# victorramirez952/tomography_3d_reconstructor

Hardware: AMD Instinct MI355X
Metric: Mvoxels/s (SDF+MC) on 1024^3 ellipsoid stack; achieved HBM GB/s vs peak (higher is better)
Workload: dtype f64

## Files before the change

### include/tomo_hip.h

```cpp
#ifndef TOMO_HIP_H
#define TOMO_HIP_H

#include <stddef.h>
#include <stdint.h>

#ifdef __cplusplus
extern "C" {
#endif

#define TOMO_OK 0
#define TOMO_E_ARG (-1)
#define TOMO_E_LAUNCH (-2)
#define TOMO_E_SIZE (-3)
#define TOMO_E_WORKSPACE (-4)

int tomo_abi_version(void);
const char *tomo_error_string(int code);
int tomo_host_mc_cell(const float *h_v, double iso, int8_t *h_tris, int *h_uses_centre);
double tomo_host_mc_edge_offset(double va, double vb);
void tomo_host_mc_centre_offset(const double *h_v8, double *h_out3);

int tomo_host_checksum(const void *h_data, int64_t nbytes, int nthreads, uint64_t *h_out);
int tomo_host_checksum_impl(const void *h_data, int64_t nbytes, int nthreads, int impl, uint64_t *h_out);
int64_t tomo_host_checksum_chunk_bytes(void);
// ... 57 lines not shown
int tomo_field_signs(const float *field, int Nz, int Ny, int Nx, int64_t pitch, int xorg, double iso, int z_begin,
                     int z_end, unsigned long long *signs, uint8_t *gcls, void *stream);

int tomo_mc_classify(const unsigned long long *signs, const uint8_t *gcls, int Nz, int Ny, int Nx, int xorg,
                     unsigned long long *seg_act, uint32_t *seg_cnt, void *stream);
int tomo_mc_scan_segments(const uint32_t *seg_cnt, int64_t nseg, uint32_t *seg_aoff, unsigned long long *totals,
                          void *workspace, int64_t workspace_bytes, void *stream);
int64_t tomo_mc_scan_workspace_bytes(int64_t n);
int tomo_mc_scan(const uint32_t *counts, int64_t n, uint32_t *off_a, uint32_t *off_b, uint32_t *nz_ids,
                 unsigned long long *totals, void *workspace, int64_t workspace_bytes, void *stream);
int tomo_mc_list(int Nz, int Ny, int Nx, int xorg, const uint32_t *seg_aoff, const unsigned long long *seg_act,
                 unsigned long long *vox_key, void *stream);
int tomo_mc_eval(const float *field, int Nz, int Ny, int Nx, int64_t pitch, int xorg, double iso,
                 const unsigned long long *vox_key, int64_t na, uint32_t *vox_counts, uint8_t *vox_flags, void *stream);
int tomo_mc_list_capped(int Nz, int Ny, int Nx, int xorg, const uint32_t *seg_aoff, const unsigned long long *seg_act,
                        unsigned long long *vox_key, int64_t cap, void *stream);
int tomo_mc_eval_capped(const float *field, int Nz, int Ny, int Nx, int64_t pitch, int xorg, double iso,
                        const unsigned long long *vox_key, int64_t cap, const unsigned long long *na_dev,
                        uint32_t *vox_counts, uint8_t *vox_flags, void *stream);
int tomo_mc_emit(const float *field, int Nz, int Ny, int Nx, int64_t pitch, int xorg, double iso,
                 const unsigned long long *vox_key, int64_t na, const unsigned long long *seg_act,
                 const uint32_t *seg_aoff, const uint32_t *vox_voff, const uint32_t *vox_foff, const uint8_t *vox_flags,
                 int z_offset, unsigned long long *vkey, float *vpos, int32_t *faces, unsigned long long *totals,
                 void *stream);

int tomo_mc_first_touch(const float *field, int Nz, int Ny, int Nx, int64_t pitch, int xorg, double iso,
                        const unsigned long long *vox_key, int64_t na, const unsigned long long *seg_act,
                        const uint32_t *seg_aoff, const uint32_t *vox_voff, const uint8_t *vox_flags, int mode,
                        uint32_t *created, const uint32_t *base, int32_t *ft_rank, unsigned long long *totals, void *stream);

int tomo_mc3_list(int Nz, int Ny, int Nx, int xorg, const uint32_t *seg_cnt, const unsigned long long *seg_act,
                  uint32_t *seg_blk, uint32_t *seg_aoff, unsigned long long *vox_key, int64_t cap, unsigned long long *tot,
                  void *stream);
int tomo_mc3_eval(const float *field, int Nz, int Ny, int Nx, int64_t pitch, int xorg, double iso,
                  const unsigned long long *vox_key, int64_t cap, const unsigned long long *tot, int z_offset,
                  uint32_t *vox_loc, int32_t *vox_til, uint8_t *vox_flags, uint16_t *vox_used, float *vox_f3, float *vox_c3,
                  uint32_t *blk3, void *stream);
int64_t tomo_mc3_slice_table_words(int Nz, int Ny);
int64_t tomo_mc3_sort_segments(int Nz, int Ny);
int tomo_mc3_scan(int Nz, int Ny, int Nx, int xorg, const uint32_t *seg_aoff, const uint32_t *vox_loc, int64_t cap,
                  uint32_t *blk3, uint32_t *slice_tab, unsigned long long *tot, int64_t cap_v, int64_t cap_f, void *stream);
int tomo_mc3_vertices(int Nz, int Ny, int Nx, int xorg, const unsigned long long *vox_key, int64_t cap,
                      const unsigned long long *tot, const uint32_t *vox_loc, const uint8_t *vox_flags, const float *vox_f3,
                      const float *vox_c3, const uint32_t *blk3, const uint32_t *slice_tab, int z_offset, int shift,
                      const double *cum, int64_t ncum, const double *adj, int64_t nadj, float mm_y, float mm_x, float *vrec,
                      uint32_t *keys, uint32_t *idx, void *stream);
int64_t tomo_mc3_sort_workspace_bytes(int64_t cap_v, int64_t nseg);
int tomo_mc3_sort_rank_top(const float *vrec, uint32_t *keys, uint32_t *idx, int64_t cap_v, int Nz, int Ny, const uint32_t *slice_tab,
                           unsigned long long *tot, float *uniq, int32_t *table, void *workspace, int64_t workspace_bytes,
                           float z_top, void *stream);
int tomo_mc3_sort_rank_fused(const float *vrec, const uint32_t *keys, int64_t cap_v, int Nz, int Ny, uint32_t *slice_tab,
                             unsigned long long *tot, float *uniq, int32_t *table, float z_top, void *stream);
int tomo_mc3_faces(int Nz, int Ny, int Nx, int xorg, const unsigned long long *vox_key, int64_t cap, unsigned long long *tot,
                   const unsigned long long *seg_act, const uint32_t *seg_aoff, const uint32_t *vox_loc, const int32_t *vox_til,
                   const uint16_t *vox_used, const uint32_t *blk3, const int32_t *table, int64_t *faces, int64_t cap_f,
                   void *stream);

int tomo_vertex_finalize(float *vpos, int64_t nv, int shift, const double *cum, int64_t ncum,
                         const double *adj, int64_t nadj, float mm_y, float mm_x, void *stream);
int64_t tomo_mesh_unique_workspace_bytes(int64_t nv);
int tomo_mesh_unique(const float *vpos, int64_t nv, float *uniq, int32_t *rank, unsigned long long *totals,
                     void *workspace, int64_t workspace_bytes, void *stream);
int tomo_mesh_lookup(const float *uniq, int64_t nu, const float *query, int64_t nq, int32_t *out,
                     unsigned long long *missing, void *stream);
int tomo_slab_top_rows(const float *uniq, const unsigned long long *tot, int64_t cap_v, int64_t cap, float *msg, void *stream);
int tomo_slab_lookup(const float *uniq, const unsigned long long *tot, int64_t cap_v, const float *msg, int64_t cap,
// ... 42 lines not shown
```

### tomography_3d_reconstructor_amd/_lib.py

```python
import ctypes
import os
import subprocess

_HERE = os.path.dirname(os.path.abspath(__file__))
SO_PATH = os.environ.get("TOMO_LIB") or os.path.join(_HERE, "libtomo_hip.so")
CSRC = os.path.join(_HERE, "csrc")

_c_i = ctypes.c_int
_c_i64 = ctypes.c_int64
_c_p = ctypes.c_void_p
_c_d = ctypes.c_double
_c_f = ctypes.c_float

SIGNATURES = {
    "tomo_abi_version": (_c_i, []),
    "tomo_error_string": (ctypes.c_char_p, [_c_i]),
    "tomo_host_mc_cell": (_c_i, [_c_p, _c_d, _c_p, _c_p]),
    "tomo_host_mc_edge_offset": (_c_d, [_c_d, _c_d]),
    "tomo_host_mc_centre_offset": (None, [_c_p, _c_p]),
    "tomo_host_checksum": (_c_i, [_c_p, _c_i64, _c_i, _c_p]),
    "tomo_host_checksum_impl": (_c_i, [_c_p, _c_i64, _c_i, _c_i, _c_p]),
    "tomo_host_checksum_chunk_bytes": (_c_i64, []),
    "tomo_host_checksum_part": (_c_i, [_c_p, _c_i64, _c_i64, _c_i, _c_i, _c_p]),
    "tomo_host_checksum_fold": (_c_i, [_c_p, _c_i64, _c_i64, _c_p]),
# ... 24 lines not shown
    "tomo_pack_close_ends": (_c_i, [_c_p, _c_p, _c_i, _c_i, _c_i, _c_p, _c_p]),
    "tomo_pack_bits_pair": (_c_i, [_c_p, _c_p, _c_i, _c_p, _c_p, _c_i, _c_i, _c_i, _c_p]),
    "tomo_slab_edges": (_c_i, [_c_p, _c_p, _c_i, _c_i, _c_i, _c_i, _c_p, _c_p, _c_i, _c_i, _c_p, _c_p, _c_p, _c_i, _c_p, _c_p, _c_p, _c_p,
                               _c_i, _c_p, _c_p]),
    "tomo_pack_close_range": (_c_i, [_c_p, _c_p, _c_i, _c_i, _c_i, _c_i, _c_i, _c_p, _c_p, _c_i, _c_i, _c_p]),
    "tomo_close_ends_workspace_words": (_c_i64, [_c_i, _c_i, _c_i]),
    "tomo_close_ends_scan": (_c_i, [_c_p, _c_i, _c_i, _c_i, _c_p, _c_p]),
    "tomo_close_ends_gp": (_c_i, [_c_p, _c_i, _c_i, _c_i, _c_p, _c_p, _c_p]),
    "tomo_morph_pass": (_c_i, [_c_p, _c_p, _c_i, _c_i, _c_i, _c_i, _c_p]),
    "tomo_morph_fused": (_c_i, [_c_p, _c_p, _c_i, _c_i, _c_i, ctypes.c_uint32, _c_i, _c_p]),
    "tomo_smooth": (_c_i, [_c_p, _c_p, _c_i, _c_i, _c_i, _c_i, _c_i, _c_p]),
    "tomo_extend_bits": (_c_i, [_c_p, _c_p, _c_i, _c_i, _c_i, _c_i, _c_p]),
    "tomo_field_fill": (_c_i, [_c_p, _c_p, _c_i, _c_i, _c_i, _c_i, _c_i, _c_p, _c_p, _c_p]),
    "tomo_field_fill_bits": (_c_i, [_c_p, _c_p, _c_i, _c_i, _c_i, _c_i, _c_p, _c_p, _c_p]),
    "tomo_field_span_bytes": (_c_i64, [_c_i, _c_i, _c_i, _c_i]),
    "tomo_field_fill_bits_sparse": (_c_i, [_c_p, _c_p, _c_i, _c_i, _c_i, _c_i, _c_p, _c_p, _c_p, _c_p]),
    "tomo_sign_rows": (_c_i64, [_c_i]),
    "tomo_field_signs_fused": (_c_i, [_c_i]),
    "tomo_sign_buffer_words": (_c_i64, [_c_i, _c_i, _c_i, _c_i]),
    "tomo_field_signs": (_c_i, [_c_p, _c_i, _c_i, _c_i, _c_i64, _c_i, _c_d, _c_i, _c_i, _c_p, _c_p, _c_p]),
    "tomo_mc_classify": (_c_i, [_c_p, _c_p, _c_i, _c_i, _c_i, _c_i, _c_p, _c_p, _c_p]),
    "tomo_mc_scan_segments": (_c_i, [_c_p, _c_i64, _c_p, _c_p, _c_p, _c_i64, _c_p]),
    "tomo_mc_scan_workspace_bytes": (_c_i64, [_c_i64]),
    "tomo_mc_scan": (_c_i, [_c_p, _c_i64, _c_p, _c_p, _c_p, _c_p, _c_p, _c_i64, _c_p]),
    "tomo_mc_list": (_c_i, [_c_i, _c_i, _c_i, _c_i, _c_p, _c_p, _c_p, _c_p]),
    "tomo_mc_eval": (_c_i, [_c_p, _c_i, _c_i, _c_i, _c_i64, _c_i, _c_d, _c_p, _c_i64, _c_p, _c_p, _c_p]),
    "tomo_mc_list_capped": (_c_i, [_c_i, _c_i, _c_i, _c_i, _c_p, _c_p, _c_p, _c_i64, _c_p]),
    "tomo_mc_eval_capped": (_c_i, [_c_p, _c_i, _c_i, _c_i, _c_i64, _c_i, _c_d, _c_p, _c_i64, _c_p, _c_p, _c_p, _c_p]),
    "tomo_mc_emit": (_c_i, [_c_p, _c_i, _c_i, _c_i, _c_i64, _c_i, _c_d, _c_p, _c_i64, _c_p, _c_p, _c_p, _c_p, _c_p, _c_i, _c_p,
                            _c_p, _c_p, _c_p, _c_p]),
    "tomo_mc_first_touch": (_c_i, [_c_p, _c_i, _c_i, _c_i, _c_i64, _c_i, _c_d, _c_p, _c_i64, _c_p, _c_p, _c_p, _c_p, _c_i, _c_p,
                                   _c_p, _c_p, _c_p, _c_p]),
    "tomo_mc3_list": (_c_i, [_c_i, _c_i, _c_i, _c_i, _c_p, _c_p, _c_p, _c_p, _c_p, _c_i64, _c_p, _c_p]),
    "tomo_mc3_eval": (_c_i, [_c_p, _c_i, _c_i, _c_i, _c_i64, _c_i, _c_d, _c_p, _c_i64, _c_p, _c_i, _c_p, _c_p, _c_p, _c_p, _c_p,
                             _c_p, _c_p, _c_p]),
    "tomo_mc3_slice_table_words": (_c_i64, [_c_i, _c_i]),
    "tomo_mc3_sort_segments": (_c_i64, [_c_i, _c_i]),
    "tomo_mc3_scan": (_c_i, [_c_i, _c_i, _c_i, _c_i, _c_p, _c_p, _c_i64, _c_p, _c_p, _c_p, _c_i64, _c_i64, _c_p]),
    "tomo_mc3_vertices": (_c_i, [_c_i, _c_i, _c_i, _c_i, _c_p, _c_i64, _c_p, _c_p, _c_p, _c_p, _c_p, _c_p, _c_p, _c_i, _c_i,
                                 _c_p, _c_i64, _c_p, _c_i64, _c_f, _c_f, _c_p, _c_p, _c_p, _c_p]),
    "tomo_mc3_sort_workspace_bytes": (_c_i64, [_c_i64, _c_i64]),
    "tomo_mc3_sort_rank_top": (_c_i, [_c_p, _c_p, _c_p, _c_i64, _c_i, _c_i, _c_p, _c_p, _c_p, _c_p, _c_p, _c_i64, _c_f, _c_p]),
    "tomo_mc3_sort_rank_fused": (_c_i, [_c_p, _c_p, _c_i64, _c_i, _c_i, _c_p, _c_p, _c_p, _c_p, _c_f, _c_p]),
    "tomo_mc3_faces": (_c_i, [_c_i, _c_i, _c_i, _c_i, _c_p, _c_i64, _c_p, _c_p, _c_p, _c_p, _c_p, _c_p, _c_p, _c_p, _c_p, _c_i64, _c_p]),
    "tomo_vertex_finalize": (_c_i, [_c_p, _c_i64, _c_i, _c_p, _c_i64, _c_p, _c_i64, _c_f, _c_f, _c_p]),
    "tomo_mesh_unique_workspace_bytes": (_c_i64, [_c_i64]),
    "tomo_mesh_unique": (_c_i, [_c_p, _c_i64, _c_p, _c_p, _c_p, _c_p, _c_i64, _c_p]),
    "tomo_mesh_lookup": (_c_i, [_c_p, _c_i64, _c_p, _c_i64, _c_p, _c_p, _c_p]),
    "tomo_slab_top_rows": (_c_i, [_c_p, _c_p, _c_i64, _c_i64, _c_p, _c_p]),
    "tomo_slab_lookup": (_c_i, [_c_p, _c_p, _c_i64, _c_p, _c_i64, _c_p, _c_p, _c_p]),
    "tomo_slab_summary": (_c_i, [_c_p, _c_i64, _c_p, _c_p, _c_i64, _c_i64, _c_p, _c_p]),
    "tomo_slab_lookup_summary": (_c_i, [_c_p, _c_p, _c_i64, _c_p, _c_i64, _c_p, _c_i64, _c_i64, _c_p, _c_p, _c_p]),
    "tomo_mc3_faces_slab": (_c_i, [_c_i, _c_i, _c_i, _c_i, _c_p, _c_i64, _c_p, _c_p, _c_p, _c_p, _c_p, _c_p, _c_p, _c_p, _c_p, _c_i64,
                                   _c_p, _c_i, _c_i, _c_p, _c_i64, _c_i64, _c_p]),
    "tomo_mesh_volume_area": (_c_i, [_c_p, _c_p, _c_i64, _c_p, _c_p]),
    "tomo_layer_colors": (_c_i, [_c_p, _c_i, _c_i64, _c_i64, _c_d, _c_d, _c_i, _c_d, _c_d, _c_i, _c_p, _c_p]),
    "tomo_mesh_edge_table_bytes": (_c_i64, [_c_i64]),
    "tomo_mesh_edges": (_c_i, [_c_p, _c_i64, _c_i64, _c_p, _c_i64, _c_p, _c_p]),
    "tomo_mesh_seam_edges": (_c_i, [_c_p, _c_i64, _c_i64, _c_i64, _c_p, _c_i64, _c_p, _c_p]),
    "tomo_mesh_seam_merge": (_c_i, [_c_p, _c_i64, _c_i64, _c_p, _c_i64, _c_p, _c_p]),
    "tomo_mesh_orient_workspace_bytes": (_c_i64, [_c_i64]),
    "tomo_mesh_orient": (_c_i, [_c_p, _c_i64, _c_i64, _c_p, _c_i64, _c_p, _c_p, _c_p]),
    "tomo_mesh_signed_volume": (_c_i, [_c_p, _c_p, _c_i64, _c_p, _c_p, _c_p]),
    "tomo_glb_pack_faces": (_c_i, [_c_p, _c_i64, _c_p, _c_p, _c_p, _c_i, _c_p]),
    "tomo_glb_pack_positions": (_c_i, [_c_p, _c_i, _c_i64, _c_p, _c_p, _c_p]),
    "tomo_mesh_vertex_normals_workspace_bytes": (_c_i64, [_c_i64, _c_i64]),
# ... 49 lines not shown
```

### tomography_3d_reconstructor_amd/csrc/mc.hip

```cpp
#include <cstring>
#include <cstdlib>
#include "tomo_common.h"
#include <rocprim/rocprim.hpp>

#define MC_LUT_QUAL __device__ const
#define MC_FN __device__ static inline
#include "mc_cell.h"

#define SEG 256
#define KEY_XBITS 20
static_assert(KEY_XBITS + 2 == TOMO_KEY_ROW_SHIFT, "key layout shared with mesh.hip");

struct McGrid {
    int Nz, Ny, Nx;
    int64_t pitch;
    int xorg;
    int segs_per_row;
    double iso;
};

typedef float float4u __attribute__((ext_vector_type(4), aligned(4)));
typedef float float2u __attribute__((ext_vector_type(2), aligned(4)));
typedef float float3u __attribute__((ext_vector_type(3), aligned(4)));
typedef int int3u __attribute__((ext_vector_type(3), aligned(4)));
// ... 27 lines not shown
    const int Y = divmod_pos(task, g.Ny, &tz);
    const int s = divmod_pos(tz, g.segs_per_row, &zq);
    const int Z = z_begin + (int)zq;
    const int X0 = s * SEG + lane * 4 - SEG_SHIFT - g.xorg;
    const int64_t NyP = tomo_sign_rows_dev(g.Ny);
    const float *row = field + ((int64_t)Z * g.Ny + Y) * g.pitch + g.xorg;
    float v[4];
#pragma unroll
    for (int k = 0; k < 4; k++) v[k] = (X0 + k >= 0 && X0 + k < g.Nx) ? row[X0 + k] : 0.0f;
    u64 b0 = __ballot((double)v[0] > g.iso), b1 = __ballot((double)v[1] > g.iso);
    u64 b2 = __ballot((double)v[2] > g.iso), b3 = __ballot((double)v[3] > g.iso);
    if (lane < 4)
        signs[((((int64_t)Z * g.segs_per_row + s) * NyP) + Y) * 4 + lane] = lane == 0 ? b0 : (lane == 1 ? b1 : (lane == 2 ? b2 : b3));
}

struct Rec4 { u64 b[4]; };

__device__ static inline Rec4 load_rec(const u64 *__restrict__ signs, int64_t idx)
{
    const ulonglong2 *q = (const ulonglong2 *)(signs + idx * 4);
    ulonglong2 lo = q[0], hi = q[1];
    Rec4 r; r.b[0] = lo.x; r.b[1] = lo.y; r.b[2] = hi.x; r.b[3] = hi.y;
    return r;
}

__device__ static inline Rec4 rec_of(const u64 *__restrict__ signs, int64_t idx, int gc)
{
    if (gc == 2) return load_rec(signs, idx);
    Rec4 r;
    r.b[0] = r.b[1] = r.b[2] = r.b[3] = gc ? ~0ull : 0ull;
    return r;
}

__global__ __launch_bounds__(256) void mc_classify_bits_kernel(const u64 *__restrict__ signs,
                                                               const unsigned char *__restrict__ gcls, const McGrid g,
                                                               int64_t ntasks, u64 *__restrict__ seg_act,
                                                               u32 *__restrict__ seg_cnt)
{
    const int64_t task = (int64_t)blockIdx.x * blockDim.x + threadIdx.x;
    if (task >= ntasks) return;
    int64_t tz, zq;
    const int Y = divmod_pos(task, g.Ny, &tz);
    const int s = divmod_pos(tz, g.segs_per_row, &zq);
    const int Z = (int)zq;
    const int S = g.segs_per_row;
    const int Yn = Y + 1 < g.Ny ? Y + 1 : g.Ny - 1, Z1 = Z + 1 < g.Nz ? Z + 1 : g.Nz - 1;
    const int Xbase = s * SEG - SEG_SHIFT - g.xorg;
    const int64_t segi = ((int64_t)Z * g.Ny + Y) * S + s;
    if (Xbase >= g.Nx || Xbase + SEG <= 0) { seg_cnt[segi] = 0u; return; }
    const bool has_next = s + 1 < S;
    const int64_t NyP = tomo_sign_rows_dev(g.Ny);
    const int64_t ia = ((int64_t)Z * S + s) * NyP + Y, ib = ((int64_t)Z * S + s) * NyP + Yn;
    const int64_t ic = ((int64_t)Z1 * S + s) * NyP + Y, id = ((int64_t)Z1 * S + s) * NyP + Yn;
    const int64_t G = NyP >> 4;
    const int64_t qa = ((int64_t)Z * G + (Y >> 4)) * S + s, qb = ((int64_t)Z * G + (Yn >> 4)) * S + s;
    const int64_t qc = ((int64_t)Z1 * G + (Y >> 4)) * S + s, qd = ((int64_t)Z1 * G + (Yn >> 4)) * S + s;
    const int ga = gcls[qa], gb = gcls[qb], gc = gcls[qc], gd = gcls[qd];
    const int na = has_next ? gcls[qa + 1] : ga, nb = has_next ? gcls[qb + 1] : gb;
    const int nc = has_next ? gcls[qc + 1] : gc, nd = has_next ? gcls[qd + 1] : gd;
    if (ga != 2 && ga == gb && ga == gc && ga == gd && na == ga && nb == ga && nc == ga && nd == ga) {
        seg_cnt[segi] = 0u;
        return;
    }
    Rec4 R[4] = {rec_of(signs, ia, ga), rec_of(signs, ib, gb), rec_of(signs, ic, gc), rec_of(signs, id, gd)};
    u64 nx0[4];
    nx0[0] = has_next ? (na == 2 ? signs[(ia + NyP) * 4] & 1ull : (u64)na) : 0ull;
    nx0[1] = has_next ? (nb == 2 ? signs[(ib + NyP) * 4] & 1ull : (u64)nb) : 0ull;
    nx0[2] = has_next ? (nc == 2 ? signs[(ic + NyP) * 4] & 1ull : (u64)nc) : 0ull;
    nx0[3] = has_next ? (nd == 2 ? signs[(id + NyP) * 4] & 1ull : (u64)nd) : 0ull;
    u64 act[4];
    u64 any_nonzero = 0;
#pragma unroll
    for (int k = 0; k < 4; k++) {
        int lo = Xbase + k < 0 ? (-(Xbase + k) + 3) / 4 : 0;
        int hi = (g.Nx - 1 - Xbase - k) >= 0 ? (g.Nx - 1 - Xbase - k) / 4 : -1;
        if (hi > 63) hi = 63;
        u64 vmask = 0;
        if (hi >= lo) vmask = (hi - lo == 63) ? ~0ull : (((1ull << (hi - lo + 1)) - 1ull) << lo);
        int dl = g.Nx - 1 - Xbase - k;
        u64 lastm = (dl >= 0 && (dl & 3) == 0 && (dl >> 2) < 64) ? (1ull << (dl >> 2)) : 0ull;
        u64 any = 0, all = ~0ull;
#pragma unroll
        for (int r = 0; r < 4; r++) {
            u64 cur = R[r].b[k];
            u64 nxt = k < 3 ? R[r].b[k + 1] : ((R[r].b[0] >> 1) | (nx0[r] << 63));
            nxt = (nxt & ~lastm) | (cur & lastm);
            any |= cur | nxt;
            all &= cur & nxt;
        }
        act[k] = any & ~all & vmask;
        any_nonzero |= act[k];
    }
    seg_cnt[segi] = any_nonzero ? (u32)(__popcll(act[0]) + __popcll(act[1]) + __popcll(act[2]) + __popcll(act[3])) : 0u;
    if (any_nonzero) {
        ulonglong2 *o = (ulonglong2 *)(seg_act + segi * 4);
        o[0] = make_ulonglong2(act[0], act[1]);
        o[1] = make_ulonglong2(act[2], act[3]);
    }
}

static inline int make_grid(McGrid &g, const float *field, int Nz, int Ny, int Nx, int64_t pitch, int xorg, double iso)
{
    if (!field || Nz < 2 || Ny < 2 || Nx < 2 || pitch < Nx + xorg) return TOMO_E_ARG;
    if (Nx >= (1 << KEY_XBITS)) return TOMO_E_SIZE;
    g.Nz = Nz; g.Ny = Ny; g.Nx = Nx; g.pitch = pitch; g.xorg = xorg; g.iso = iso;
    g.segs_per_row = (int)tomo_mc_segments_per_row(Nx, xorg);
    return TOMO_OK;
}

TOMO_API int tomo_field_signs(const float *field, int Nz, int Ny, int Nx, int64_t pitch, int xorg, double iso,
                              int z_begin, int z_end, unsigned long long *signs, uint8_t *gcls, void *stream)
{
    McGrid g;
    int rc = make_grid(g, field, Nz, Ny, Nx, pitch, xorg, iso);
    if (rc) return rc;
    if (!signs || !gcls || z_begin < 0 || z_end > Nz || z_begin > z_end) return TOMO_E_ARG;
    {
        const int64_t per_slice = (tomo_sign_rows(Ny) >> 4) * g.segs_per_row;
        if (z_end > z_begin && hipMemsetAsync(gcls + z_begin * per_slice, 2, (size_t)((z_end - z_begin) * per_slice),
                                              (hipStream_t)stream) != hipSuccess)
            return TOMO_E_LAUNCH;
    }
    int64_t ntasks = (int64_t)(z_end - z_begin) * g.segs_per_row * Ny;
    if (ntasks == 0) return TOMO_OK;
    int64_t blocks = ceil_div64(ntasks, 4);
    if (blocks > 0x7fffffff) return TOMO_E_SIZE;
    hipLaunchKernelGGL(field_signs_kernel, dim3((unsigned)blocks), dim3(256), 0, (hipStream_t)stream, field, g, z_begin,
                       ntasks, (u64 *)signs);
    return tomo_status();
}

TOMO_API int tomo_mc_classify(const unsigned long long *signs, const uint8_t *gcls, int Nz, int Ny, int Nx, int xorg,
                              unsigned long long *seg_act, uint32_t *seg_cnt, void *stream)
{
    if (!signs || !gcls || !seg_act || !seg_cnt || Nz < 2 || Ny < 2 || Nx < 2) return TOMO_E_ARG;
    if (Nx >= (1 << KEY_XBITS)) return TOMO_E_SIZE;
    McGrid g; g.Nz = Nz; g.Ny = Ny; g.Nx = Nx; g.pitch = 0; g.xorg = xorg; g.iso = 0.0;
    g.segs_per_row = (int)tomo_mc_segments_per_row(Nx, xorg);
    int64_t nseg = (int64_t)Nz * Ny * g.segs_per_row;
    int64_t blocks = ceil_div64(nseg, 256);
    if (blocks > 0x7fffffff) return TOMO_E_SIZE;
    hipLaunchKernelGGL(mc_classify_bits_kernel, dim3((unsigned)blocks), dim3(256), 0, (hipStream_t)stream,
                       (const u64 *)signs, gcls, g, nseg, (u64 *)seg_act, seg_cnt);
    return tomo_status();
}

struct ScanPair { u32 a, b; };
struct ScanUnpack {
    __host__ __device__ rocprim::tuple<u32, u32> operator()(u32 c) const { return rocprim::make_tuple(c & 0xffffu, c >> 16); }
};
struct ScanAdd {
    __host__ __device__ rocprim::tuple<u32, u32> operator()(const rocprim::tuple<u32, u32> &x,
                                                            const rocprim::tuple<u32, u32> &y) const
    {
        return rocprim::make_tuple(rocprim::get<0>(x) + rocprim::get<0>(y), rocprim::get<1>(x) + rocprim::get<1>(y));
    }
};

__global__ void scan_finish_kernel(u32 *__restrict__ off_a, u32 *__restrict__ off_b, int64_t n, u64 *__restrict__ totals)
{
    if (threadIdx.x == 0 && blockIdx.x == 0) {
        off_a[0] = 0u;
        if (off_b) off_b[0] = 0u;
        totals[0] = off_a[n];
        totals[1] = off_b ? off_b[n] : 0ull;
        totals[2] = 0ull;
        totals[3] = 0ull;
    }
}

static size_t scan_temp_bytes(int64_t n)
{
    size_t t1 = 0, t2 = 0;
    size_t m = (size_t)(n > 0 ? n : 1);
    (void)rocprim::inclusive_scan(nullptr, t1, (u32 *)nullptr, (u32 *)nullptr, m, rocprim::plus<u32>(), (hipStream_t)0);
    auto in = rocprim::make_transform_iterator((const u32 *)nullptr, ScanUnpack());
    auto out = rocprim::make_zip_iterator(rocprim::make_tuple((u32 *)nullptr, (u32 *)nullptr));
// ... 533 lines not shown
        for (int k = 0; k < K; k++) {
            u32 ex = carry[k] + lds[k * 16 + w] + inc[k] - s[k];
            u32 *p = a + k * stride + i0;
            if (i0 + 7 < n && ((uintptr_t)p & 15) == 0) {
                uint4 lo, hi;
                lo.x = ex; ex += v[k][0]; lo.y = ex; ex += v[k][1]; lo.z = ex; ex += v[k][2]; lo.w = ex; ex += v[k][3];
                hi.x = ex; ex += v[k][4]; hi.y = ex; ex += v[k][5]; hi.z = ex; ex += v[k][6]; hi.w = ex;
                *(uint4 *)p = lo; *(uint4 *)(p + 4) = hi;
            } else {
#pragma unroll
                for (int j = 0; j < 8; j++) { if (i0 + j < n) p[j] = ex; ex += v[k][j]; }
            }
            carry[k] += lds[K * 16 + k];
            wide[k] += lds[K * 16 + k];
        }
        __syncthreads();
    }
#pragma unroll
    for (int k = 0; k < K; k++) total_out[k] = wide[k];
}

__global__ __launch_bounds__(1024) void mc3_scan_seg_kernel(u32 *__restrict__ seg_blk, int64_t nblk, u64 *__restrict__ tot)
{
    __shared__ u32 lds[17];
    u64 total;
    scan_small_inplace<1>(seg_blk, 0, nblk, &total, lds);
    if (threadIdx.x == 0) {
        tot[0] = total;
        tot[1] = tot[2] = tot[4] = tot[5] = tot[6] = tot[7] = 0ull;
        tot[3] = total > 0xffffffffull ? 1ull : 0ull;
    }
}

__global__ __launch_bounds__(MC3_BLK) void mc3_list_kernel(const McGrid g, const u32 *__restrict__ seg_cnt,
                                                           const u32 *__restrict__ seg_blk, const u64 *__restrict__ seg_act,
                                                           int64_t nseg, u32 *__restrict__ seg_aoff, u64 *__restrict__ vox_key,
                                                           u32 cap, u64 *__restrict__ tot)
{
    __shared__ u32 wsum[4];
    const int lane = threadIdx.x & 63, w = threadIdx.x >> 6;
    const int64_t seg = (int64_t)blockIdx.x * MC3_BLK + threadIdx.x;
    const u32 cnt = seg < nseg ? seg_cnt[seg] : 0u;
    const u32 inc = wave_inclusive_scan(cnt);
    if (lane == 63) wsum[w] = inc;
    __syncthreads();
    u32 o = seg_blk[blockIdx.x] + inc - cnt;
    for (int k = 0; k < w; k++) o += wsum[k];
    if (seg >= nseg) return;
    seg_aoff[seg] = o;
    if (seg == nseg - 1) seg_aoff[nseg] = o + cnt;
    if (cnt == 0) return;
    if ((u64)o + cnt > (u64)cap || tot[0] > (u64)cap) {
        if (o <= cap) atomicOr((unsigned long long *)&tot[3], 1ull);
        return;
    }
    int64_t row;
    const int s = divmod_pos(seg, g.segs_per_row, &row);
    const ulonglong2 *q = (const ulonglong2 *)(seg_act + seg * 4);
    const ulonglong2 lo = q[0], hi = q[1];
    const u64 b0 = lo.x, b1 = lo.y, b2 = hi.x, b3 = hi.y;
    const int Xs = s * SEG - SEG_SHIFT - g.xorg;
    u64 any = b0 | b1 | b2 | b3;
    while (any) {
        const int L = __ffsll((long long)any) - 1;
        any &= any - 1;
        const int X0 = Xs + 4 * L;
        if ((b0 >> L) & 1ull) vox_key[o++] = make_key(row, X0, 0);
        if ((b1 >> L) & 1ull) vox_key[o++] = make_key(row, X0 + 1, 0);
        if ((b2 >> L) & 1ull) vox_key[o++] = make_key(row, X0 + 2, 0);
        if ((b3 >> L) & 1ull) vox_key[o++] = make_key(row, X0 + 3, 0);
    }
}

TOMO_API int tomo_mc3_list(int Nz, int Ny, int Nx, int xorg, const uint32_t *seg_cnt, const unsigned long long *seg_act,
                           uint32_t *seg_blk, uint32_t *seg_aoff, unsigned long long *vox_key, int64_t cap,
                           unsigned long long *tot, void *stream)
{
    if (Nz < 2 || Ny < 2 || Nx < 2 || !seg_cnt || !seg_act || !seg_blk || !seg_aoff || !vox_key || !tot) return TOMO_E_ARG;
    if (cap <= 0 || cap >= 0x1fffffffll) return TOMO_E_SIZE;
    if (Nx >= (1 << KEY_XBITS)) return TOMO_E_SIZE;
    McGrid g; g.Nz = Nz; g.Ny = Ny; g.Nx = Nx; g.pitch = 0; g.xorg = xorg; g.iso = 0.0;
    g.segs_per_row = (int)tomo_mc_segments_per_row(Nx, xorg);
    const int64_t nseg = (int64_t)Nz * Ny * g.segs_per_row, nblk = ceil_div64(nseg, MC3_BLK);
    if (nblk > 0x7fffffff) return TOMO_E_SIZE;
    hipStream_t s = (hipStream_t)stream;
    hipLaunchKernelGGL(mc3_segsum_kernel, dim3((unsigned)ceil_div64(nblk, 4)), dim3(256), 0, s, seg_cnt, nseg, seg_blk, nblk);
    hipLaunchKernelGGL(mc3_scan_seg_kernel, dim3(1), dim3(1024), 0, s, seg_blk, nblk, (u64 *)tot);
    hipLaunchKernelGGL(mc3_list_kernel, dim3((unsigned)nblk), dim3(MC3_BLK), 0, s, g, seg_cnt, (const u32 *)seg_blk,
                       (const u64 *)seg_act, nseg, seg_aoff, (u64 *)vox_key, (u32)cap, (u64 *)tot);
    return tomo_status();
}

__global__ __launch_bounds__(MC3_BLK) void mc3_eval_kernel(const float *__restrict__ field, const McGrid g,
                                                           const u64 *__restrict__ vox_key, int64_t cap,
                                                           const u64 *__restrict__ tot, int z_offset,
                                                           u32 *__restrict__ vox_loc, int32_t *__restrict__ vox_til,
                                                           uint8_t *__restrict__ vox_flags, uint16_t *__restrict__ vox_used,
                                                           float *__restrict__ vox_f3, float *__restrict__ vox_c3,
                                                           u32 *__restrict__ blk3, int64_t nblk)
{
    __shared__ u32 wsum[4];
    const int lane = threadIdx.x & 63, w = threadIdx.x >> 6;
    const int64_t i = (int64_t)blockIdx.x * MC3_BLK + threadIdx.x;
    const u64 na = tot[0];
    const bool live = i < cap && (u64)i < na && na <= (u64)cap;
    u32 packed = 0;
    if (live) {
        Cell c;
        load_cell(field, g, vox_key[i], c);
        int ntri = 0;
        int32_t til = 0;
        u32 used = 0;
        if (c.cell_ok && c.index != 0 && c.index != 255) {
            const McTiling t = mc_cell_tiling(c.v, c.index);
            ntri = t.ntri;
            if (t.centre) c.flags |= 8;
            til = (int32_t)(((intptr_t)t.tris - (intptr_t)LUT_TILING1) * 16 + ntri);
            const int ix = c.index;
#define BICH(a, b) ((u32)(((ix >> (a)) ^ (ix >> (b))) & 1))
            used = BICH(0, 1) | BICH(1, 2) << 1 | BICH(2, 3) << 2 | BICH(3, 0) << 3 | BICH(4, 5) << 4 | BICH(5, 6) << 5 | BICH(6, 7) << 6 |
                   BICH(7, 4) << 7 | BICH(0, 4) << 8 | BICH(1, 5) << 9 | BICH(2, 6) << 10 | BICH(3, 7) << 11 | (t.centre ? 1u << 12 : 0u);
#undef BICH
            if (ntri == 0) used = 0;
// ... 378 lines not shown
```

### tomography_3d_reconstructor_amd/pipeline.py

```python
import math
import os
import threading
from dataclasses import dataclass

import numpy as np
import torch

from . import _lib


COUNTERS = dict.fromkeys(("na_hint_hit", "na_hint_miss", "mc3_hint_hit", "mc3_hint_miss", "mc3_sort_fused", "mc3_sort_library",
                          "mc3_exact", "mc3_general_unique", "mc3_degenerate"), 0)
NA_HINTS = os.environ.get("TOMO_NA_HINTS", "1") not in ("", "0")
_NA_HINT = {}
LIST_LIMIT = 2 ** 31
MESH_LIMIT = 2 ** 31
PACK_CLOSE_FUSED = os.environ.get("TOMO_PACK_CLOSE", "1") not in ("", "0")
FIELD_FROM_BITS = True
FIELD_SPARSE = os.environ.get("TOMO_FIELD_SPARSE", "0") not in ("", "0")


def _stream():
    return torch.cuda.current_stream().cuda_stream

# ... 439 lines not shown
    _free = {}

    def __init__(self, t):
        t = t.reshape(-1)
        self._key = (str(t.device), threading.get_ident(), int(t.numel()))
        pool = PendingDownload._free.setdefault(self._key, [])
        self._host = pool.pop() if pool else torch.empty(t.numel(), dtype=torch.int64, pin_memory=True)
        self._host.copy_(t, non_blocking=True)
        self._event = torch.cuda.Event()
        self._event.record(torch.cuda.current_stream(t.device))

    def wait(self, timeout_s=None):
        if timeout_s is None:
            self._event.synchronize()
        else:
            wait_event(self._event, timeout_s, "the counters of a pass")
        out = self._host.tolist()
        PendingDownload._free[self._key].append(self._host)
        self._host = None
        return out


class Mc3Surface:

    def __init__(self, f, slice_depths, mm_per_pixel_y, mm_per_pixel_x, add_padding=True, z_offset=0, z_top=None, tot=None):
        self.field, self.z_offset = f, int(z_offset)
        self.z_top = float("nan") if z_top is None else float(z_top)
        self.hint_key = (f.Nz, f.Ny, f.Nx, self.z_offset)
        self._depth = _depth_args(slice_depths, add_padding, f.data.device)
        self._mm = (float(np.float32(mm_per_pixel_y)), float(np.float32(mm_per_pixel_x)))
        self.tot = torch.empty(8, dtype=torch.int64, device=f.data.device) if tot is None else tot
        self.uniq = self.table = self.faces_final = None
        self.nv = self.nf = self.na = 0
        self.deferred = False
        self._pending = None

    def classify(self):
        L, f, dev = _lib.lib(), self.field, self.field.data.device
        if f.signs is None or f.signs_level != 0.5:
            if f.sparse:
                raise _lib.TomoError("a sparse field holds floats only near the 0.5 surface")
            field_signs(f, 0.5)
        nseg = f.Nz * f.Ny * L.tomo_mc_segments_per_row(f.Nx, f.xorg)
        self.seg_act = torch.empty(nseg * 4, dtype=torch.int64, device=dev)
        self.seg_cnt = torch.empty(nseg, dtype=torch.int32, device=dev)
        _lib.check(L.tomo_mc_classify(_p(f.signs), _p(f.gcls), f.Nz, f.Ny, f.Nx, f.xorg, _p(self.seg_act), _p(self.seg_cnt), _stream()),
                   "tomo_mc_classify")
        self.seg_blk = torch.empty((nseg + 255) // 256, dtype=torch.int32, device=dev)
        self.seg_aoff = torch.empty(nseg + 1, dtype=torch.int32, device=dev)

    def build_list(self, cap):
        f, self.cap = self.field, cap
        self.vox_key = torch.empty(cap, dtype=torch.int64, device=f.data.device)
        _lib.check(_lib.lib().tomo_mc3_list(f.Nz, f.Ny, f.Nx, f.xorg, _p(self.seg_cnt), _p(self.seg_act), _p(self.seg_blk), _p(self.seg_aoff),
                                            _p(self.vox_key), cap, _p(self.tot), _stream()), "tomo_mc3_list")

    def eval_scan(self, cap_v, cap_f):
        L, f, cap, st, dev = _lib.lib(), self.field, self.cap, _stream(), self.field.data.device
        self.vox_loc = torch.empty(cap, dtype=torch.int32, device=dev)
        self.vox_til = torch.empty(cap, dtype=torch.int32, device=dev)
        self.vox_flags = torch.empty(cap, dtype=torch.uint8, device=dev)
        self.vox_used = torch.empty(cap, dtype=torch.int16, device=dev)
        self.vox_f3 = torch.empty(3 * cap, dtype=torch.float32, device=dev)
        self.vox_c3 = torch.empty(3 * cap, dtype=torch.float32, device=dev)
        self.blk3 = torch.empty(3 * ((cap + 255) // 256), dtype=torch.int32, device=dev)
        self.slice_tab = torch.empty(L.tomo_mc3_slice_table_words(f.Nz, f.Ny), dtype=torch.int32, device=dev)
        _lib.check(L.tomo_mc3_eval(_p(f.data), f.Nz, f.Ny, f.Nx, f.pitch, f.xorg, 0.5, _p(self.vox_key), cap, _p(self.tot), self.z_offset,
                                   _p(self.vox_loc), _p(self.vox_til), _p(self.vox_flags), _p(self.vox_used), _p(self.vox_f3),
                                   _p(self.vox_c3), _p(self.blk3), st), "tomo_mc3_eval")
        _lib.check(L.tomo_mc3_scan(f.Nz, f.Ny, f.Nx, f.xorg, _p(self.seg_aoff), _p(self.vox_loc), cap, _p(self.blk3), _p(self.slice_tab),
                                   _p(self.tot), cap_v, cap_f, st), "tomo_mc3_scan")

    def vertices_sort(self, cap_v):
        L, f, cap, tot, st, dev = _lib.lib(), self.field, self.cap, self.tot, _stream(), self.field.data.device
        cum_t, ncum, adj_t, nadj = self._depth
        self.cap_v = cap_v
        self.vrec = torch.empty((cap_v, 4), dtype=torch.float32, device=dev)
        keys = torch.empty(cap_v, dtype=torch.int32, device=dev)
        self.rows = torch.empty((cap_v, 3), dtype=torch.float32, device=dev)
        self.table = torch.empty(4 * cap, dtype=torch.int32, device=dev)
        fused = FUSED_SORT and not _MC3_LARGE.get(self.hint_key)
        idx = None if fused else torch.empty(cap_v, dtype=torch.int32, device=dev)
        _lib.check(L.tomo_mc3_vertices(f.Nz, f.Ny, f.Nx, f.xorg, _p(self.vox_key), cap, _p(tot), _p(self.vox_loc), _p(self.vox_flags),
                                       _p(self.vox_f3), _p(self.vox_c3), _p(self.blk3), _p(self.slice_tab), self.z_offset, 1, _p(cum_t), ncum,
                                       _p(adj_t), nadj, *self._mm, _p(self.vrec), _p(keys), _p(idx), st), "tomo_mc3_vertices")
        if fused:
            COUNTERS["mc3_sort_fused"] += 1
            _lib.check(L.tomo_mc3_sort_rank_fused(_p(self.vrec), _p(keys), cap_v, f.Nz, f.Ny, _p(self.slice_tab), _p(tot), _p(self.rows),
# ... 426 lines not shown
```

Before: 663,600.

## Fuse per-block segment sums into classify and skip empty blocks in MC list

The classify kernel now produces per-block active-voxel sums directly, so the separate segsum kernel and its re-read of seg_cnt are dropped. Classify also checks the coarse gcls classes for a whole block up front and exits early when the block is uniformly inside or outside. Threads are remapped so adjacent lanes handle segments from different rows. The list kernel skips blocks whose sum is zero and spreads wide segments (16 or more active voxels) across the whole wave via readlane broadcasts. This adds shared-memory and indexing complexity, and the block-level gcls pre-check is redundant work for blocks that are not uniform.

Measured after the change: 661,900. Within noise of the previous version (-0.3%).

```diff
diff --git a/include/tomo_hip.h b/include/tomo_hip.h
--- a/include/tomo_hip.h
+++ b/include/tomo_hip.h
@@ -113,6 +113,11 @@
 int tomo_mc3_list(int Nz, int Ny, int Nx, int xorg, const uint32_t *seg_cnt, const unsigned long long *seg_act,
                   uint32_t *seg_blk, uint32_t *seg_aoff, unsigned long long *vox_key, int64_t cap, unsigned long long *tot,
                   void *stream);
+int tomo_mc3_classify_sums(const unsigned long long *signs, const uint8_t *gcls, int Nz, int Ny, int Nx, int xorg,
+                           unsigned long long *seg_act, uint32_t *seg_cnt, uint32_t *seg_blk, void *stream);
+int tomo_mc3_list_from_sums(int Nz, int Ny, int Nx, int xorg, const uint32_t *seg_cnt, const unsigned long long *seg_act,
+                            uint32_t *seg_blk, uint32_t *seg_aoff, unsigned long long *vox_key, int64_t cap,
+                            unsigned long long *tot, void *stream);
 int tomo_mc3_eval(const float *field, int Nz, int Ny, int Nx, int64_t pitch, int xorg, double iso,
                   const unsigned long long *vox_key, int64_t cap, const unsigned long long *tot, int z_offset,
                   uint32_t *vox_loc, int32_t *vox_til, uint8_t *vox_flags, uint16_t *vox_used, float *vox_f3, float *vox_c3,
diff --git a/tomography_3d_reconstructor_amd/_lib.py b/tomography_3d_reconstructor_amd/_lib.py
--- a/tomography_3d_reconstructor_amd/_lib.py
+++ b/tomography_3d_reconstructor_amd/_lib.py
@@ -80,6 +80,8 @@
     "tomo_mc_first_touch": (_c_i, [_c_p, _c_i, _c_i, _c_i, _c_i64, _c_i, _c_d, _c_p, _c_i64, _c_p, _c_p, _c_p, _c_p, _c_i, _c_p,
                                    _c_p, _c_p, _c_p, _c_p]),
     "tomo_mc3_list": (_c_i, [_c_i, _c_i, _c_i, _c_i, _c_p, _c_p, _c_p, _c_p, _c_p, _c_i64, _c_p, _c_p]),
+    "tomo_mc3_classify_sums": (_c_i, [_c_p, _c_p, _c_i, _c_i, _c_i, _c_i, _c_p, _c_p, _c_p, _c_p]),
+    "tomo_mc3_list_from_sums": (_c_i, [_c_i, _c_i, _c_i, _c_i, _c_p, _c_p, _c_p, _c_p, _c_p, _c_i64, _c_p, _c_p]),
     "tomo_mc3_eval": (_c_i, [_c_p, _c_i, _c_i, _c_i, _c_i64, _c_i, _c_d, _c_p, _c_i64, _c_p, _c_i, _c_p, _c_p, _c_p, _c_p, _c_p,
                              _c_p, _c_p, _c_p]),
     "tomo_mc3_slice_table_words": (_c_i64, [_c_i, _c_i]),
diff --git a/tomography_3d_reconstructor_amd/csrc/mc.hip b/tomography_3d_reconstructor_amd/csrc/mc.hip
--- a/tomography_3d_reconstructor_amd/csrc/mc.hip
+++ b/tomography_3d_reconstructor_amd/csrc/mc.hip
@@ -83,22 +83,17 @@
     return r;
 }
 
-__global__ __launch_bounds__(256) void mc_classify_bits_kernel(const u64 *__restrict__ signs,
-                                                               const unsigned char *__restrict__ gcls, const McGrid g,
-                                                               int64_t ntasks, u64 *__restrict__ seg_act,
-                                                               u32 *__restrict__ seg_cnt)
-{
-    const int64_t task = (int64_t)blockIdx.x * blockDim.x + threadIdx.x;
-    if (task >= ntasks) return;
-    int64_t tz, zq;
-    const int Y = divmod_pos(task, g.Ny, &tz);
-    const int s = divmod_pos(tz, g.segs_per_row, &zq);
+__device__ static inline u32 classify_segment(const u64 *__restrict__ signs, const unsigned char *__restrict__ gcls,
+                                              const McGrid &g, int64_t segi, u64 *__restrict__ seg_act)
+{
+    const int S = g.segs_per_row;
+    int64_t row, zq;
+    const int s = divmod_pos(segi, S, &row);
+    const int Y = divmod_pos(row, g.Ny, &zq);
     const int Z = (int)zq;
-    const int S = g.segs_per_row;
     const int Yn = Y + 1 < g.Ny ? Y + 1 : g.Ny - 1, Z1 = Z + 1 < g.Nz ? Z + 1 : g.Nz - 1;
     const int Xbase = s * SEG - SEG_SHIFT - g.xorg;
-    const int64_t segi = ((int64_t)Z * g.Ny + Y) * S + s;
-    if (Xbase >= g.Nx || Xbase + SEG <= 0) { seg_cnt[segi] = 0u; return; }
+    if (Xbase >= g.Nx || Xbase + SEG <= 0) return 0u;
     const bool has_next = s + 1 < S;
     const int64_t NyP = tomo_sign_rows_dev(g.Ny);
     const int64_t ia = ((int64_t)Z * S + s) * NyP + Y, ib = ((int64_t)Z * S + s) * NyP + Yn;
@@ -109,10 +104,8 @@
     const int ga = gcls[qa], gb = gcls[qb], gc = gcls[qc], gd = gcls[qd];
     const int na = has_next ? gcls[qa + 1] : ga, nb = has_next ? gcls[qb + 1] : gb;
     const int nc = has_next ? gcls[qc + 1] : gc, nd = has_next ? gcls[qd + 1] : gd;
-    if (ga != 2 && ga == gb && ga == gc && ga == gd && na == ga && nb == ga && nc == ga && nd == ga) {
-        seg_cnt[segi] = 0u;
-        return;
-    }
+    if (ga != 2 && ga == gb && ga == gc && ga == gd && na == ga && nb == ga && nc == ga && nd == ga)
+        return 0u;
     Rec4 R[4] = {rec_of(signs, ia, ga), rec_of(signs, ib, gb), rec_of(signs, ic, gc), rec_of(signs, id, gd)};
     u64 nx0[4];
     nx0[0] = has_next ? (na == 2 ? signs[(ia + NyP) * 4] & 1ull : (u64)na) : 0ull;
@@ -142,11 +135,59 @@
         act[k] = any & ~all & vmask;
         any_nonzero |= act[k];
     }
-    seg_cnt[segi] = any_nonzero ? (u32)(__popcll(act[0]) + __popcll(act[1]) + __popcll(act[2]) + __popcll(act[3])) : 0u;
-    if (any_nonzero) {
-        ulonglong2 *o = (ulonglong2 *)(seg_act + segi * 4);
-        o[0] = make_ulonglong2(act[0], act[1]);
-        o[1] = make_ulonglong2(act[2], act[3]);
+    if (!any_nonzero) return 0u;
+    ulonglong2 *o = (ulonglong2 *)(seg_act + segi * 4);
+    o[0] = make_ulonglong2(act[0], act[1]);
+    o[1] = make_ulonglong2(act[2], act[3]);
+    return (u32)(__popcll(act[0]) + __popcll(act[1]) + __popcll(act[2]) + __popcll(act[3]));
+}
+
+__global__ __launch_bounds__(256) void mc_classify_bits_kernel(const u64 *__restrict__ signs,
+                                                               const unsigned char *__restrict__ gcls, const McGrid g,
+                                                               int64_t nseg, u64 *__restrict__ seg_act,
+                                                               u32 *__restrict__ seg_cnt, u32 *__restrict__ seg_blk)
+{
+    __shared__ u32 cl[256];
+    __shared__ u32 wsum[4];
+    const int t = threadIdx.x, S = g.segs_per_row;
+    const int64_t B = (int64_t)blockIdx.x * 256;
+    const int64_t last = B + 255 < nseg ? B + 255 : nseg - 1;
+    int64_t R0, R1, Za, Zb;
+    (void)divmod_pos(B, S, &R0);
+    (void)divmod_pos(last, S, &R1);
+    const int Ya = divmod_pos(R0, g.Ny, &Za), Yb = divmod_pos(R1, g.Ny, &Zb);
+    {
+        const int G = (int)(tomo_sign_rows_dev(g.Ny) >> 4);
+        const bool one = Za == Zb;
+        const int g0 = one ? Ya >> 4 : 0, g1 = one ? (Yb + 1 < g.Ny ? Yb + 1 : g.Ny - 1) >> 4 : G - 1;
+        const int ng = g1 - g0 + 1, nz = (int)((Zb + 1 < g.Nz ? Zb + 1 : g.Nz - 1) - Za) + 1;
+        const int ncand = nz * ng * S;
+        const int ref = gcls[(Za * G + g0) * S];
+        int ok = ref != 2;
+        for (int j = t; j < ncand; j += 256) {
+            const int sj = j % S, r = j / S;
+            ok &= gcls[((Za + r / ng) * G + g0 + r % ng) * S + sj] == ref;
+        }
+        if (__syncthreads_and(ok)) {
+            if (B + t < nseg) seg_cnt[B + t] = 0u;
+            if (seg_blk && t == 0) seg_blk[blockIdx.x] = 0u;
+            return;
+        }
+    }
+    const int q = 256 / S, rem = 256 - q * S;
+    int c, i;
+    if (t < rem * (q + 1)) { c = t / (q + 1); i = t - c * (q + 1); }
+    else { const int u = t - rem * (q + 1); c = rem + u / q; i = u - (c - rem) * q; }
+    const int l = c + i * S;
+    cl[l] = B + l < nseg ? classify_segment(signs, gcls, g, B + l, seg_act) : 0u;
+    __syncthreads();
+    const u32 cnt = cl[t];
+    if (B + t < nseg) seg_cnt[B + t] = cnt;
+    if (seg_blk) {
+        const u32 ws = wave_sum(cnt);
+        if ((t & 63) == 0) wsum[t >> 6] = ws;
+        __syncthreads();
+        if (t == 0) seg_blk[blockIdx.x] = wsum[0] + wsum[1] + wsum[2] + wsum[3];
     }
 }
 
@@ -181,8 +222,8 @@
     return tomo_status();
 }
 
-TOMO_API int tomo_mc_classify(const unsigned long long *signs, const uint8_t *gcls, int Nz, int Ny, int Nx, int xorg,
-                              unsigned long long *seg_act, uint32_t *seg_cnt, void *stream)
+static int mc_classify_launch(const unsigned long long *signs, const uint8_t *gcls, int Nz, int Ny, int Nx, int xorg,
+                              unsigned long long *seg_act, uint32_t *seg_cnt, uint32_t *seg_blk, void *stream)
 {
     if (!signs || !gcls || !seg_act || !seg_cnt || Nz < 2 || Ny < 2 || Nx < 2) return TOMO_E_ARG;
     if (Nx >= (1 << KEY_XBITS)) return TOMO_E_SIZE;
@@ -192,8 +233,21 @@
     int64_t blocks = ceil_div64(nseg, 256);
     if (blocks > 0x7fffffff) return TOMO_E_SIZE;
     hipLaunchKernelGGL(mc_classify_bits_kernel, dim3((unsigned)blocks), dim3(256), 0, (hipStream_t)stream,
-                       (const u64 *)signs, gcls, g, nseg, (u64 *)seg_act, seg_cnt);
+                       (const u64 *)signs, gcls, g, nseg, (u64 *)seg_act, seg_cnt, seg_blk);
     return tomo_status();
+}
+
+TOMO_API int tomo_mc_classify(const unsigned long long *signs, const uint8_t *gcls, int Nz, int Ny, int Nx, int xorg,
+                              unsigned long long *seg_act, uint32_t *seg_cnt, void *stream)
+{
+    return mc_classify_launch(signs, gcls, Nz, Ny, Nx, xorg, seg_act, seg_cnt, nullptr, stream);
+}
+
+TOMO_API int tomo_mc3_classify_sums(const unsigned long long *signs, const uint8_t *gcls, int Nz, int Ny, int Nx, int xorg,
+                                    unsigned long long *seg_act, uint32_t *seg_cnt, uint32_t *seg_blk, void *stream)
+{
+    if (!seg_blk) return TOMO_E_ARG;
+    return mc_classify_launch(signs, gcls, Nz, Ny, Nx, xorg, seg_act, seg_cnt, seg_blk, stream);
 }
 
 struct ScanPair { u32 a, b; };
@@ -793,6 +847,14 @@
     }
 }
 
+#define MC3_LIST_WIDE 16u
+
+__device__ static inline u64 bcast64(u64 v, int src)
+{
+    const u32 lo = (u32)__builtin_amdgcn_readlane((int)(u32)v, src), hi = (u32)__builtin_amdgcn_readlane((int)(u32)(v >> 32), src);
+    return ((u64)hi << 32) | lo;
+}
+
 __global__ __launch_bounds__(MC3_BLK) void mc3_list_kernel(const McGrid g, const u32 *__restrict__ seg_cnt,
                                                            const u32 *__restrict__ seg_blk, const u64 *__restrict__ seg_act,
                                                            int64_t nseg, u32 *__restrict__ seg_aoff, u64 *__restrict__ vox_key,
@@ -801,27 +863,53 @@
     __shared__ u32 wsum[4];
     const int lane = threadIdx.x & 63, w = threadIdx.x >> 6;
     const int64_t seg = (int64_t)blockIdx.x * MC3_BLK + threadIdx.x;
+    const u64 na = tot[0];
+    const u32 base = seg_blk[blockIdx.x];
+    const u32 bsum = ((int64_t)blockIdx.x + 1 < (int64_t)gridDim.x ? seg_blk[blockIdx.x + 1] : (u32)na) - base;
+    if (bsum == 0) {
+        if (seg < nseg) seg_aoff[seg] = base;
+        if (seg == nseg - 1) seg_aoff[nseg] = base;
+        return;
+    }
     const u32 cnt = seg < nseg ? seg_cnt[seg] : 0u;
     const u32 inc = wave_inclusive_scan(cnt);
     if (lane == 63) wsum[w] = inc;
     __syncthreads();
-    u32 o = seg_blk[blockIdx.x] + inc - cnt;
+    u32 o = base + inc - cnt;
     for (int k = 0; k < w; k++) o += wsum[k];
-    if (seg >= nseg) return;
-    seg_aoff[seg] = o;
+    if (seg < nseg) seg_aoff[seg] = o;
     if (seg == nseg - 1) seg_aoff[nseg] = o + cnt;
-    if (cnt == 0) return;
-    if ((u64)o + cnt > (u64)cap || tot[0] > (u64)cap) {
+    bool fits = cnt != 0;
+    if (fits && ((u64)o + cnt > (u64)cap || na > (u64)cap)) {
         if (o <= cap) atomicOr((unsigned long long *)&tot[3], 1ull);
-        return;
-    }
-    int64_t row;
-    const int s = divmod_pos(seg, g.segs_per_row, &row);
-    const ulonglong2 *q = (const ulonglong2 *)(seg_act + seg * 4);
-    const ulonglong2 lo = q[0], hi = q[1];
-    const u64 b0 = lo.x, b1 = lo.y, b2 = hi.x, b3 = hi.y;
-    const int Xs = s * SEG - SEG_SHIFT - g.xorg;
-    u64 any = b0 | b1 | b2 | b3;
+        fits = false;
+    }
+    int64_t row = 0;
+    int Xs = 0;
+    u64 b0 = 0, b1 = 0, b2 = 0, b3 = 0;
+    if (fits) {
+        const int s = divmod_pos(seg, g.segs_per_row, &row);
+        const ulonglong2 *q = (const ulonglong2 *)(seg_act + seg * 4);
+        const ulonglong2 lo = q[0], hi = q[1];
+        b0 = lo.x; b1 = lo.y; b2 = hi.x; b3 = hi.y;
+        Xs = s * SEG - SEG_SHIFT - g.xorg;
+    }
+    u64 wide = __ballot(fits && cnt >= MC3_LIST_WIDE);
+    const u64 below = (1ull << lane) - 1ull;
+    while (wide) {
+        const int src = __ffsll((long long)wide) - 1;
+        wide &= wide - 1;
+        const u64 c0 = bcast64(b0, src), c1 = bcast64(b1, src), c2 = bcast64(b2, src), c3 = bcast64(b3, src);
+        const u64 r = (u64)bcast64((u64)row, src);
+        const int X0 = __builtin_amdgcn_readlane(Xs, src) + 4 * lane;
+        u32 p = (u32)__builtin_amdgcn_readlane((int)o, src)
+                + (u32)(__popcll(c0 & below) + __popcll(c1 & below) + __popcll(c2 & below) + __popcll(c3 & below));
+        if ((c0 >> lane) & 1ull) vox_key[p++] = make_key((int64_t)r, X0, 0);
+        if ((c1 >> lane) & 1ull) vox_key[p++] = make_key((int64_t)r, X0 + 1, 0);
+        if ((c2 >> lane) & 1ull) vox_key[p++] = make_key((int64_t)r, X0 + 2, 0);
+        if ((c3 >> lane) & 1ull) vox_key[p++] = make_key((int64_t)r, X0 + 3, 0);
+    }
+    u64 any = fits && cnt < MC3_LIST_WIDE ? b0 | b1 | b2 | b3 : 0ull;
     while (any) {
         const int L = __ffsll((long long)any) - 1;
         any &= any - 1;
@@ -833,9 +921,9 @@
     }
 }
 
-TOMO_API int tomo_mc3_list(int Nz, int Ny, int Nx, int xorg, const uint32_t *seg_cnt, const unsigned long long *seg_act,
+static int mc3_list_launch(int Nz, int Ny, int Nx, int xorg, const uint32_t *seg_cnt, const unsigned long long *seg_act,
                            uint32_t *seg_blk, uint32_t *seg_aoff, unsigned long long *vox_key, int64_t cap,
-                           unsigned long long *tot, void *stream)
+                           unsigned long long *tot, bool have_sums, void *stream)
 {
     if (Nz < 2 || Ny < 2 || Nx < 2 || !seg_cnt || !seg_act || !seg_blk || !seg_aoff || !vox_key || !tot) return TOMO_E_ARG;
     if (cap <= 0 || cap >= 0x1fffffffll) return TOMO_E_SIZE;
@@ -845,11 +933,26 @@
     const int64_t nseg = (int64_t)Nz * Ny * g.segs_per_row, nblk = ceil_div64(nseg, MC3_BLK);
     if (nblk > 0x7fffffff) return TOMO_E_SIZE;
     hipStream_t s = (hipStream_t)stream;
-    hipLaunchKernelGGL(mc3_segsum_kernel, dim3((unsigned)ceil_div64(nblk, 4)), dim3(256), 0, s, seg_cnt, nseg, seg_blk, nblk);
+    if (!have_sums)
+        hipLaunchKernelGGL(mc3_segsum_kernel, dim3((unsigned)ceil_div64(nblk, 4)), dim3(256), 0, s, seg_cnt, nseg, seg_blk, nblk);
     hipLaunchKernelGGL(mc3_scan_seg_kernel, dim3(1), dim3(1024), 0, s, seg_blk, nblk, (u64 *)tot);
     hipLaunchKernelGGL(mc3_list_kernel, dim3((unsigned)nblk), dim3(MC3_BLK), 0, s, g, seg_cnt, (const u32 *)seg_blk,
                        (const u64 *)seg_act, nseg, seg_aoff, (u64 *)vox_key, (u32)cap, (u64 *)tot);
     return tomo_status();
+}
+
+TOMO_API int tomo_mc3_list(int Nz, int Ny, int Nx, int xorg, const uint32_t *seg_cnt, const unsigned long long *seg_act,
+                           uint32_t *seg_blk, uint32_t *seg_aoff, unsigned long long *vox_key, int64_t cap,
+                           unsigned long long *tot, void *stream)
+{
+    return mc3_list_launch(Nz, Ny, Nx, xorg, seg_cnt, seg_act, seg_blk, seg_aoff, vox_key, cap, tot, false, stream);
+}
+
+TOMO_API int tomo_mc3_list_from_sums(int Nz, int Ny, int Nx, int xorg, const uint32_t *seg_cnt, const unsigned long long *seg_act,
+                                     uint32_t *seg_blk, uint32_t *seg_aoff, unsigned long long *vox_key, int64_t cap,
+                                     unsigned long long *tot, void *stream)
+{
+    return mc3_list_launch(Nz, Ny, Nx, xorg, seg_cnt, seg_act, seg_blk, seg_aoff, vox_key, cap, tot, true, stream);
 }
 
 __global__ __launch_bounds__(MC3_BLK) void mc3_eval_kernel(const float *__restrict__ field, const McGrid g,
diff --git a/tomography_3d_reconstructor_amd/pipeline.py b/tomography_3d_reconstructor_amd/pipeline.py
--- a/tomography_3d_reconstructor_amd/pipeline.py
+++ b/tomography_3d_reconstructor_amd/pipeline.py
@@ -495,7 +495,7 @@
         self.tot = torch.empty(8, dtype=torch.int64, device=f.data.device) if tot is None else tot
         self.uniq = self.table = self.faces_final = None
         self.nv = self.nf = self.na = 0
-        self.deferred = False
+        self.deferred = self._blk_sums = False
         self._pending = None
 
     def classify(self):
@@ -507,16 +507,20 @@
         nseg = f.Nz * f.Ny * L.tomo_mc_segments_per_row(f.Nx, f.xorg)
         self.seg_act = torch.empty(nseg * 4, dtype=torch.int64, device=dev)
         self.seg_cnt = torch.empty(nseg, dtype=torch.int32, device=dev)
-        _lib.check(L.tomo_mc_classify(_p(f.signs), _p(f.gcls), f.Nz, f.Ny, f.Nx, f.xorg, _p(self.seg_act), _p(self.seg_cnt), _stream()),
-                   "tomo_mc_classify")
         self.seg_blk = torch.empty((nseg + 255) // 256, dtype=torch.int32, device=dev)
+        _lib.check(L.tomo_mc3_classify_sums(_p(f.signs), _p(f.gcls), f.Nz, f.Ny, f.Nx, f.xorg, _p(self.seg_act), _p(self.seg_cnt),
+                                            _p(self.seg_blk), _stream()), "tomo_mc3_classify_sums")
+        self._blk_sums = True
         self.seg_aoff = torch.empty(nseg + 1, dtype=torch.int32, device=dev)
 
     def build_list(self, cap):
         f, self.cap = self.field, cap
         self.vox_key = torch.empty(cap, dtype=torch.int64, device=f.data.device)
-        _lib.check(_lib.lib().tomo_mc3_list(f.Nz, f.Ny, f.Nx, f.xorg, _p(self.seg_cnt), _p(self.seg_act), _p(self.seg_blk), _p(self.seg_aoff),
-                                            _p(self.vox_key), cap, _p(self.tot), _stream()), "tomo_mc3_list")
+        L = _lib.lib()
+        fn, what = (L.tomo_mc3_list_from_sums, "tomo_mc3_list_from_sums") if self._blk_sums else (L.tomo_mc3_list, "tomo_mc3_list")
+        self._blk_sums = False
+        _lib.check(fn(f.Nz, f.Ny, f.Nx, f.xorg, _p(self.seg_cnt), _p(self.seg_act), _p(self.seg_blk), _p(self.seg_aoff),
+                      _p(self.vox_key), cap, _p(self.tot), _stream()), what)
 
     def eval_scan(self, cap_v, cap_f):
         L, f, cap, st, dev = _lib.lib(), self.field, self.cap, _stream(), self.field.data.device
```
